# zrlhahaha/Direct12PBRRenderer

Hardware: AMD Instinct MI355X
Metric: shaded Mpixel/s at 4K G-buffer (full deferred frame: clustered shade + bloom + auto-exposure + ACES) (higher is better)
Workload: dtype f32

## Files before the change

direct12pbrrenderer_amd/csrc/bloom.hip:

```cpp
#include <type_traits>
#include "pbr_internal.hpp"
#include "pbr_device.hpp"

using namespace pbr;

__constant__ float c_gauss[9] = {0.0148f, 0.0459f, 0.1050f, 0.1941f, 0.2803f, 0.1941f, 0.1050f, 0.0459f, 0.0148f};

__device__ __forceinline__ float4 to4(F4 v) { return make_float4(v.x, v.y, v.z, v.w); }
__device__ __forceinline__ F4 from4(float4 v) { return f4(v.x, v.y, v.z, v.w); }

struct OutRect { int x0, y0, x1, y1, ox, oy, pitch; };
constexpr int PF_MAX_RECTS = 5;
struct OutRects {
    int n, ox, oy, pitch;
    int x0[PF_MAX_RECTS], y0[PF_MAX_RECTS], x1[PF_MAX_RECTS], y1[PF_MAX_RECTS], tiles_x[PF_MAX_RECTS], first[PF_MAX_RECTS + 1];
};
__global__ __launch_bounds__(256) void k_bloom_prefilter(const pbr_half* __restrict__ hdr, int w, int h, int pitch,
                                                           pbr_half* __restrict__ out, OutRect rc,
                                                           float tx, float ty, float threshold, float knee) {
    const int x = rc.x0 + blockIdx.x * 64 + threadIdx.x;
    const int y = rc.y0 + blockIdx.y * 4 + threadIdx.y;
    if (x >= rc.x1 || y >= rc.y1) return;
    const float u = (float)x * tx, v = (float)y * ty;
    const float ox[5] = {0.0f, -1.0f, -1.0f, 1.0f, 1.0f};
// ... 272 lines not shown
    t.c00 = r0[x0];
    if (MODE != M_SAME) {
        const H4* r1 = reinterpret_cast<const H4*>(in) + (size_t)y1 * iw;
        t.c10 = r0[x1]; t.c01 = r1[x0]; t.c11 = r1[x1];
    }
    return t;
}
template <int MODE>
__device__ __forceinline__ float4 finish_tap2(const Tap2& t, float fx, float fy) {
    if (MODE == M_SAME) return to4(h4f(t.c00));
    const float wx0 = 1.0f - fx, wy0 = 1.0f - fy;
    const F4 top = fma4(h4f(t.c10), fx, h4f(t.c00) * wx0);
    const F4 bot = fma4(h4f(t.c11), fx, h4f(t.c01) * wx0);
    return to4(fma4(bot, fy, top * wy0));
}

typedef _Float16 half4v __attribute__((ext_vector_type(4)));
typedef _Float16 half2v __attribute__((ext_vector_type(2)));
typedef float float2v __attribute__((ext_vector_type(2)));
__device__ __forceinline__ half2v round_h2(float a, float b) {
    asm volatile("" : "+v"(a), "+v"(b));
    float2v f; f.x = a; f.y = b;
    return __builtin_convertvector(f, half2v);
}
__device__ __forceinline__ half4v round_h4(F4 v) {
    half4v r;
    r.x = to_half_rn(v.x); r.y = to_half_rn(v.y); r.z = to_half_rn(v.z); r.w = to_half_rn(v.w);
    return r;
}

__device__ __forceinline__ V3 h3f(H4 h) { return v3((float)h.x, (float)h.y, (float)h.z); }
__device__ __forceinline__ V3 fma3(V3 a, float s, V3 b) { return v3(__builtin_fmaf(a.x, s, b.x), __builtin_fmaf(a.y, s, b.y), __builtin_fmaf(a.z, s, b.z)); }
template <int MODE>
__device__ __forceinline__ float4 finish_tap2_rgb(const Tap2& t, float fx, float fy) {
    if (MODE == M_SAME) return make_float4((float)t.c00.x, (float)t.c00.y, (float)t.c00.z, 0.0f);
    const float wx0 = 1.0f - fx, wy0 = 1.0f - fy;
    const V3 top = fma3(h3f(t.c10), fx, h3f(t.c00) * wx0);
    const V3 bot = fma3(h3f(t.c11), fx, h3f(t.c01) * wx0);
    const V3 r = fma3(bot, fy, top * wy0);
    return make_float4(r.x, r.y, r.z, 0.0f);
}
__device__ __forceinline__ V3 gauss9_rgb(const float4* c) {
    V3 v = v3(0.0f, 0.0f, 0.0f);
#pragma unroll
    for (int i = 0; i < 9; i++) { const float4 e = c[i]; v = fma3(v3(e.x, e.y, e.z), c_gauss[i], v); }
    return v;
}
__device__ __forceinline__ float gauss9_const(float c) {
    float v = 0.0f;
#pragma unroll
    for (int i = 0; i < 9; i++) v = __builtin_fmaf(c, c_gauss[i], v);
    return v;
}

struct TailRect { int tx0, ty0, mx0, my0, mx1, my1, bx, by, hx0, hy0, hx1, hy1; };

template <int MODE, bool DUAL, int TAIL, int TH, int NT>
__global__ __launch_bounds__(NT, 4) void k_blur_hv(const pbr_half* __restrict__ in, int iw, int ih,
                                                 const pbr_half* __restrict__ in2,
                                                 pbr_half* __restrict__ out, int ow, int oh, int out_pitch,
                                                 int tiles_x, int n_tiles,
                                                 TailRect tr, float min_log, float inv_range,
                                                 uint32_t* __restrict__ hist) {
    constexpr int TW = 64, SW = TW + 8, SR = TH + 8;
    constexpr int NW = NT / 64;
    constexpr int PER_T = SR / NW;
    constexpr int PER_O = TH / NW;
    static_assert(SR % NW == 0 && TH % NW == 0 && PER_T * 8 <= 64, "rows must split evenly over the waves; one halo tap per lane");
    __shared__ float4 sLine[DUAL ? 2 : 1][NW][SW];
    __shared__ H4 sT[SR][TW];
    __shared__ uint32_t sh_hist[TAIL == 2 ? NW : 1][TAIL == 2 ? PBR_HISTOGRAM_BINS : 1];
    const int t = threadIdx.x, lane = t & 63;
    const int wv = __builtin_amdgcn_readfirstlane(t >> 6);
    if (TAIL == 2) {
        for (int i = t; i < NW * PBR_HISTOGRAM_BINS; i += NT) (&sh_hist[0][0])[i] = 0u;
    }
    const size_t a_at = MODE == M_UP ? (size_t)min(tr.my0 >> 1, ih - 1) * iw + min(tr.mx0 >> 1, iw - 1) : (size_t)0;
    float alpha_h = gauss9_const((float)reinterpret_cast<const H4*>(in)[a_at].w);
    if (DUAL) alpha_h = alpha_h + gauss9_const((float)reinterpret_cast<const H4*>(in2)[(size_t)min(tr.my0, oh - 1) * ow + min(tr.mx0, ow - 1)].w);
    const h16 alpha_t = to_half_rn(alpha_h);
    const float alpha_v = gauss9_const((float)alpha_t);
    for (int tile = blockIdx.x; tile < n_tiles; tile += gridDim.x) {
    const int x0 = (tr.tx0 + tile % tiles_x) * TW, y0 = (tr.ty0 + tile / tiles_x) * TH;
    const int x = x0 + lane;
    H4 hdr_in[PER_O];
    const bool in_mx = TAIL != 0 && x >= tr.mx0 && x < tr.mx1;
    if (TAIL != 0) {
#pragma unroll
        for (int k = 0; k < PER_O; k++) {
            const int y = y0 + wv + NW * k;
            if (in_mx && y >= tr.my0 && y < tr.my1) hdr_in[k] = *reinterpret_cast<const H4*>(out + 4 * ((size_t)(y - tr.by) * out_pitch + (x - tr.bx)));
        }
    }
    const int r0 = wv * PER_T;
    const bool has_halo = lane < PER_T * 8;
    const int hk = lane >> 3, hc = 64 + (lane & 7);
    float4* line = sLine[0][wv];
    float4* line2 = sLine[DUAL ? 1 : 0][wv];
    auto wave_sync = [] {
        __builtin_amdgcn_fence(__ATOMIC_RELEASE, "wavefront");
        __builtin_amdgcn_wave_barrier();
        __builtin_amdgcn_fence(__ATOMIC_ACQUIRE, "wavefront");
    };
    {
        Tap2 htap;
        H4 up[DUAL ? PER_T : 1], hup;
        float fx, hfx, hfy = 0.0f;
        float4 smp[PER_T];
        int ax0, ax1, bx0, bx1;
        tap1d<MODE>(x0 - 4 + lane, iw, ax0, ax1, fx);
        tap1d<MODE>(x0 - 4 + hc, iw, bx0, bx1, hfx);
        const int sx = clampi(x0 - 4 + lane, 0, ow - 1), shx = clampi(x0 - 4 + hc, 0, ow - 1);
        const int first = y0 - 4 + r0;
        const bool shared_rows = MODE == M_UP && first >= 1 && first + PER_T - 1 <= oh - 2;
        if (MODE == M_UP && shared_rows) {
            constexpr int NR = PER_T / 2 + 2;
            const int base = (first >> 1) - 1 + (first & 1);
            V3 hrow[NR];
            const float wx0 = 1.0f - fx;
#pragma unroll
            for (int j = 0; j < NR; j++) {
                const H4* row = reinterpret_cast<const H4*>(in) + (size_t)min(base + j, ih - 1) * iw;
                const H4 c0 = row[ax0], c1 = row[ax1];
                hrow[j] = fma3(h3f(c1), fx, h3f(c0) * wx0);
            }
            auto blend = [&](auto parity) {
                constexpr int P = decltype(parity)::value;
#pragma unroll
                for (int k = 0; k < PER_T; k++) {
                    constexpr int dummy = 0; (void)dummy;
                    const int odd = (P + k) & 1;
                    const int i0 = (P + k + 1) / 2 - P;
                    const float fyk = odd ? 0.25f : 0.75f, wy0 = 1.0f - fyk;
                    const V3 r = fma3(hrow[i0 + 1], fyk, hrow[i0] * wy0);
                    smp[k] = make_float4(r.x, r.y, r.z, 0.0f);
                }
            };
            if (first & 1) blend(std::integral_constant<int, 1>{}); else blend(std::integral_constant<int, 0>{});
#pragma unroll
            for (int k = 0; k < PER_T; k++)
                if (DUAL) up[k] = reinterpret_cast<const H4*>(in2)[(size_t)(first + k) * ow + sx];
        } else {
            Tap2 taps[PER_T];
            float fy[PER_T];
#pragma unroll
            for (int k = 0; k < PER_T; k++) {
                const int jj = clampi(first + k, 0, oh - 1);
                int ay0, ay1;
                tap1d<MODE>(jj, ih, ay0, ay1, fy[k]);
                taps[k] = load_tap2<MODE>(in, iw, ax0, ax1, ay0, ay1);
                if (DUAL) up[k] = reinterpret_cast<const H4*>(in2)[(size_t)jj * ow + sx];
            }
#pragma unroll
            for (int k = 0; k < PER_T; k++) smp[k] = finish_tap2_rgb<MODE>(taps[k], fx, fy[k]);
        }
        if (has_halo) {
            const int jj = clampi(first + hk, 0, oh - 1);
            int ay0, ay1;
            tap1d<MODE>(jj, ih, ay0, ay1, hfy);
            htap = load_tap2<MODE>(in, iw, bx0, bx1, ay0, ay1);
            if (DUAL) hup = reinterpret_cast<const H4*>(in2)[(size_t)jj * ow + shx];
        }
#pragma unroll
        for (int k = 0; k < PER_T; k++) {
            line[lane] = smp[k];
            if (DUAL) line2[lane] = make_float4((float)up[k].x, (float)up[k].y, (float)up[k].z, 0.0f);
            if (has_halo && hk == k) {
                line[hc] = finish_tap2_rgb<MODE>(htap, hfx, hfy);
                if (DUAL) line2[hc] = make_float4((float)hup.x, (float)hup.y, (float)hup.z, 0.0f);
            }
            wave_sync();
            V3 g = gauss9_rgb(line + lane);
            if (DUAL) g = g + gauss9_rgb(line2 + lane);
            wave_sync();
            H4 th;
            th.x = to_half_rn(g.x); th.y = to_half_rn(g.y); th.z = to_half_rn(g.z); th.w = alpha_t;
            sT[r0 + k][lane] = th;
        }
    }
    __syncthreads();
#pragma unroll
    for (int k = 0; k < PER_O; k++) {
        const int r = wv + NW * k, y = y0 + r;
        if (x >= ow || y >= oh) continue;
        V3 a3 = v3(0.0f, 0.0f, 0.0f);
#pragma unroll
        for (int i = 0; i < 9; i++) a3 = fma3(h3f(sT[r + i][lane]), c_gauss[i], a3);
        const F4 a = f4(a3.x, a3.y, a3.z, alpha_v);
        if (TAIL == 0) {
            store_h4(out + 4 * ((size_t)y * out_pitch + x), a);
        } else {
            if (!(in_mx && y >= tr.my0 && y < tr.my1)) continue;
            const half4v a0 = round_h4(a);
            const F4 s = h4f(hdr_in[k]);
            H4 o;
            o.x = to_half_rn(s.x + (float)a0.x); o.y = to_half_rn(s.y + (float)a0.y); o.z = to_half_rn(s.z + (float)a0.z); o.w = to_half_rn(s.w + (float)a0.w);
            *reinterpret_cast<H4*>(out + 4 * ((size_t)(y - tr.by) * out_pitch + (x - tr.bx))) = o;
            if (TAIL == 2) {
                if (x >= tr.hx0 && x < tr.hx1 && y >= tr.hy0 && y < tr.hy1)
                    atomicAdd(&sh_hist[wv][luminance_bin_exact((float)o.x, (float)o.y, (float)o.z, min_log, inv_range)], 1u);
            }
        }
    }
    if (tile + (int)gridDim.x < n_tiles) __syncthreads();
    }
    if (TAIL == 2) {
        __syncthreads();
        for (int i = t; i < PBR_HISTOGRAM_BINS; i += NT) {
            uint32_t sum = 0;
#pragma unroll
            for (int w2 = 0; w2 < NW; w2++) sum += sh_hist[w2][i];
            if (sum) atomicAdd(&hist[i], sum);
        }
    }
}

__device__ __forceinline__ H4 ld_h4(const void* base, uint32_t byte_off) {
    return *reinterpret_cast<const H4*>(reinterpret_cast<const char*>(base) + byte_off);
}
__device__ __forceinline__ void pair_tap_up(const pbr_half* __restrict__ in, int iw, int cm, int c0, int cp, int ay0, int ay1, float fy,
                                            V3& even, V3& odd) {
    const uint32_t ra = (uint32_t)(ay0 * iw) * 8u, rb = (uint32_t)(ay1 * iw) * 8u, om = (uint32_t)cm * 8u, o0 = (uint32_t)c0 * 8u, op = (uint32_t)cp * 8u;
    const V3 am = h3f(ld_h4(in, ra + om)), a0 = h3f(ld_h4(in, ra + o0)), ap = h3f(ld_h4(in, ra + op));
    const V3 bm = h3f(ld_h4(in, rb + om)), b0 = h3f(ld_h4(in, rb + o0)), bp = h3f(ld_h4(in, rb + op));
    const float wy0 = 1.0f - fy;
    even = fma3(fma3(b0, 0.75f, bm * 0.25f), fy, fma3(a0, 0.75f, am * 0.25f) * wy0);
    odd = fma3(fma3(bp, 0.25f, b0 * 0.75f), fy, fma3(ap, 0.25f, a0 * 0.75f) * wy0);
}
__device__ __forceinline__ void gauss9_pair(const float2* e, float& ge, float& go) {
    const float s[10] = {e[0].x, e[0].y, e[1].x, e[1].y, e[2].x, e[2].y, e[3].x, e[3].y, e[4].x, e[4].y};
    float a = 0.0f, b = 0.0f;
#pragma unroll
    for (int i = 0; i < 9; i++) { a = __builtin_fmaf(s[i], c_gauss[i], a); b = __builtin_fmaf(s[i + 1], c_gauss[i], b); }
    ge = a; go = b;
}

#ifdef PBR_DEBUG_KNOBS
#ifdef PBR_BLOOM_TIMING
__device__ unsigned long long g_tail_stamp[8 * 4096];
#define TSTAMP(i) do { if (TAIL == 2 && t == 0 && tile == (int)blockIdx.x + PBR_BLOOM_TIMING * (int)gridDim.x && blockIdx.x < 4096) g_tail_stamp[blockIdx.x * 8 + (i)] = __builtin_readcyclecounter(); } while (0)
#define TWAIT_VM() asm volatile("s_waitcnt vmcnt(0)" ::: "memory")
extern "C" int pbr_debug_tail_stamps(unsigned long long* host, int n) { return (int)hipMemcpyFromSymbol(host, HIP_SYMBOL(g_tail_stamp), sizeof(unsigned long long) * n); }
#else
#define TSTAMP(i) do {} while (0)
#define TWAIT_VM() do {} while (0)
#endif
template <bool DUAL, int TAIL, int TH>
__global__ __launch_bounds__(512, TH == 16 ? 6 : 4) void k_blur_up_wide(const pbr_half* __restrict__ in, int iw, int ih,
                                                          const pbr_half* __restrict__ in2,
                                                          pbr_half* __restrict__ out, int ow, int oh, int out_pitch,
                                                          int tiles_x, int n_tiles,
                                                          TailRect tr, float min_log, float inv_range,
                                                          uint32_t* __restrict__ hist) {
    constexpr int TW = 128, NP = TW / 2 + 4, SR = TH + 8, NT = 512, NW = NT / 64;
    constexpr int PER_T = SR / NW;
    constexpr int PER_O = TH / 4;
    static_assert(SR % NW == 0 && TH % 4 == 0 && PER_T * 4 <= 64, "rows must split evenly over the waves; one halo pair per lane");
    __shared__ float2 sLine[DUAL ? 2 : 1][NW][3][NP];
    __shared__ H4 sT[SR][TW];
    __shared__ uint32_t sh_hist[TAIL == 2 ? NW : 1][TAIL == 2 ? PBR_HISTOGRAM_BINS : 1];
    const int t = threadIdx.x, lane = t & 63;
    const int wv = __builtin_amdgcn_readfirstlane(t >> 6);
    const int vc = t & 127, vg = __builtin_amdgcn_readfirstlane(t >> 7);
    if (TAIL == 2) {
        for (int i = t; i < NW * PBR_HISTOGRAM_BINS; i += NT) (&sh_hist[0][0])[i] = 0u;
    }
    const size_t a_at = (size_t)min(tr.my0 >> 1, ih - 1) * iw + min(tr.mx0 >> 1, iw - 1);
    float alpha_h = gauss9_const((float)reinterpret_cast<const H4*>(in)[a_at].w);
    if (DUAL) alpha_h = alpha_h + gauss9_const((float)reinterpret_cast<const H4*>(in2)[(size_t)min(tr.my0, oh - 1) * ow + min(tr.mx0, ow - 1)].w);
    const h16 alpha_t = to_half_rn(alpha_h);
    const float alpha_v = gauss9_const((float)alpha_t);
    const float a0w = (float)to_half_rn(alpha_v);
    auto wave_sync = [] {
        __builtin_amdgcn_fence(__ATOMIC_RELEASE, "wavefront");
        __builtin_amdgcn_wave_barrier();
        __builtin_amdgcn_fence(__ATOMIC_ACQUIRE, "wavefront");
    };
    for (int tile = blockIdx.x; tile < n_tiles; tile += gridDim.x) {
    const int x0 = (tr.tx0 + tile % tiles_x) * TW, y0 = (tr.ty0 + tile / tiles_x) * TH;
    const int xv = x0 + vc, rbase = vg * PER_O;
    TSTAMP(0);
    H4 hdr_in[PER_O];
    const bool in_mx = TAIL != 0 && xv >= tr.mx0 && xv < tr.mx1;
    char* const hdr_row0 = reinterpret_cast<char*>(out) + (ptrdiff_t)(y0 + rbase - tr.by) * out_pitch * 8;
    const uint32_t hdr_x = (uint32_t)(xv - tr.bx) * 8u;
    const size_t hdr_pitch = (size_t)out_pitch * 8u;
    const int r0 = wv * PER_T, first = y0 - 4 + r0;
// ... 287 lines not shown
    }
    __syncthreads();
    {
        H4 win[PER_O + 8];
#pragma unroll
        for (int i = 0; i < PER_O + 8; i++) win[i] = sT[rbase + i][vc];
#pragma unroll
        for (int k = 0; k < PER_O; k++) {
            const int y = y0 + rbase + k;
            if (xv >= ow || y >= oh) continue;
            V3 a3 = v3(0.0f, 0.0f, 0.0f);
#pragma unroll
            for (int i = 0; i < 9; i++) a3 = fma3(h3f(win[k + i]), c_gauss[i], a3);
            const F4 a = f4(a3.x, a3.y, a3.z, alpha_v);
            if (TAIL == 0) {
                store_h4(out + 4 * ((size_t)y * out_pitch + xv), a);
            } else {
                if (!(in_mx && y >= tr.my0 && y < tr.my1)) continue;
                const half2v a01 = round_h2(a3.x, a3.y);
                const h16 a2 = to_half_rn(a3.z);
                const F4 s = h4f(hdr_in[k]);
                struct alignas(8) O4 { half2v lo, hi; } o;
                o.lo = round_h2(s.x + (float)a01.x, s.y + (float)a01.y);
                o.hi = round_h2(s.z + (float)a2, s.w + a0w);
                *reinterpret_cast<O4*>(hdr_row0 + k * hdr_pitch + hdr_x) = o;
                if (TAIL == 2) {
                    if (xv >= tr.hx0 && xv < tr.hx1 && y >= tr.hy0 && y < tr.hy1)
                        atomicAdd(&sh_hist[wv][luminance_bin_exact((float)o.lo.x, (float)o.lo.y, (float)o.hi.x, min_log, inv_range)], 1u);
                }
            }
        }
    }
    if (tile + (int)gridDim.x < n_tiles) __syncthreads();
    }
    if (TAIL == 2) {
        __syncthreads();
        for (int i = t; i < PBR_HISTOGRAM_BINS; i += NT) {
            uint32_t sum = 0;
#pragma unroll
            for (int w2 = 0; w2 < NW; w2++) sum += sh_hist[w2][i];
            if (sum) atomicAdd(&hist[i], sum);
        }
    }
}

static int blur_h_rows(uint32_t ow, uint32_t oh) {
    const uint64_t row_blocks = (uint64_t)((ow + 255) / 256) * oh;
    int rows = (int)(row_blocks / 2048);
    return rows < 1 ? 1 : (rows > HB_MAX_ROWS ? HB_MAX_ROWS : rows);
}

static bool exact_half(uint32_t n) { return (n & 1u) == 0u && n <= 8192u; }
static bool force_staged() { static const bool v = pbr::knob_set("PBR_BLOOM_STAGED"); return v; }

template <int MODE, bool DUAL, int TAIL>
static pbr_status launch_hv(pbr_ctx* ctx, const pbr_half* in, uint32_t iw, uint32_t ih, const pbr_half* in2,
                            pbr_half* out, uint32_t ow, uint32_t oh, uint32_t out_pitch,
                            const uint32_t* rect, float min_log, float inv_range, uint32_t* hist,
                            const uint32_t* merge_rect = nullptr, const uint32_t* buf_origin = nullptr) {
    TailRect tr;
    tr.hx0 = rect ? (int)rect[0] : 0; tr.hy0 = rect ? (int)rect[1] : 0;
    tr.hx1 = rect ? (int)(rect[0] + rect[2]) : 0; tr.hy1 = rect ? (int)(rect[1] + rect[3]) : 0;
    tr.mx0 = merge_rect ? (int)merge_rect[0] : 0; tr.my0 = merge_rect ? (int)merge_rect[1] : 0;
    tr.mx1 = merge_rect ? (int)(merge_rect[0] + merge_rect[2]) : (int)ow; tr.my1 = merge_rect ? (int)(merge_rect[1] + merge_rect[3]) : (int)oh;
    tr.bx = buf_origin ? (int)buf_origin[0] : 0; tr.by = buf_origin ? (int)buf_origin[1] : 0;
    static const int hist_blocks = pbr::knob_int("PBR_BLOOM_HIST_BLOCKS", 1024);
    auto even_blocks = [](int n_tiles) { const int per = (n_tiles + hist_blocks - 1) / hist_blocks; return (n_tiles + per - 1) / per; };
    if constexpr (MODE == M_UP) {
        static const int wide_forced = pbr::knob_int("PBR_BLOOM_WIDE", -1);
#ifdef PBR_DEBUG_KNOBS
        static const int wide_th = pbr::knob_int("PBR_BLOOM_WIDE_TH", 32);
#endif
        const int wtx0 = tr.mx0 / 128, wty0 = tr.my0 / 32;
        const int wtiles_x = (tr.mx1 + 127) / 128 - wtx0, wn = wtiles_x * ((tr.my1 + 31) / 32 - wty0);
        if (wide_forced >= 0 ? wide_forced == 1 : (wn >= 400 && !ctx->bloom_shader_order)) {
            tr.tx0 = wtx0; tr.ty0 = wty0;
#ifdef PBR_DEBUG_KNOBS
            static const bool poly_off = pbr::knob_int("PBR_BLOOM_POLY", 1) == 0;
            if (poly_off && wide_th == 16) {
                tr.ty0 = tr.my0 / 16;
                const int wn16 = wtiles_x * ((tr.my1 + 15) / 16 - tr.ty0);
                hipLaunchKernelGGL((k_blur_up_wide<DUAL, TAIL, 16>), dim3(TAIL == 2 ? even_blocks(wn16) : wn16), dim3(512), 0, ctx->stream,
                                   in, (int)iw, (int)ih, in2, out, (int)ow, (int)oh, (int)out_pitch, wtiles_x, wn16, tr, min_log, inv_range, hist);
                return launched(ctx, "k_blur_up_wide<16>");
            }
            if (poly_off) {
                hipLaunchKernelGGL((k_blur_up_wide<DUAL, TAIL, 32>), dim3(TAIL == 2 ? even_blocks(wn) : wn), dim3(512), 0, ctx->stream,
                                   in, (int)iw, (int)ih, in2, out, (int)ow, (int)oh, (int)out_pitch, wtiles_x, wn, tr, min_log, inv_range, hist);
                return launched(ctx, "k_blur_up_wide");
            }
#endif
            hipLaunchKernelGGL((k_blur_up_poly<DUAL, TAIL, 32>), dim3(TAIL == 2 ? even_blocks(wn) : wn), dim3(512), 0, ctx->stream,
                               in, (int)iw, (int)ih, in2, out, (int)ow, (int)oh, (int)out_pitch, wtiles_x, wn, tr, min_log, inv_range, hist);
            return launched(ctx, "k_blur_up_poly");
        }
    }
    static const int forced = pbr::knob_int("PBR_BLOOM_TILE", 0);
    const bool big = forced ? forced == 32 : (uint64_t)((tr.mx1 + 63) / 64 - tr.mx0 / 64) * ((tr.my1 + 31) / 32 - tr.my0 / 32) >= 900;
    const int th = big ? 32 : 16;
    tr.tx0 = tr.mx0 / 64; tr.ty0 = tr.my0 / th;
    const int tiles_x = (tr.mx1 + 63) / 64 - tr.tx0;
    const int n_tiles = tiles_x * ((tr.my1 + th - 1) / th - tr.ty0);
    const int blocks = TAIL == 2 ? even_blocks(n_tiles) : n_tiles;
    if (big) {
        hipLaunchKernelGGL((k_blur_hv<MODE, DUAL, TAIL, 32, 512>), dim3(blocks), dim3(512), 0, ctx->stream,
                           in, (int)iw, (int)ih, in2, out, (int)ow, (int)oh, (int)out_pitch, tiles_x, n_tiles, tr, min_log, inv_range, hist);
    } else if (forced != 16) {
        hipLaunchKernelGGL((k_blur_hv<MODE, DUAL, TAIL, 16, 512>), dim3(blocks), dim3(512), 0, ctx->stream,
                           in, (int)iw, (int)ih, in2, out, (int)ow, (int)oh, (int)out_pitch, tiles_x, n_tiles, tr, min_log, inv_range, hist);
    } else {
        hipLaunchKernelGGL((k_blur_hv<MODE, DUAL, TAIL, 16, 256>), dim3(blocks), dim3(256), 0, ctx->stream,
                           in, (int)iw, (int)ih, in2, out, (int)ow, (int)oh, (int)out_pitch, tiles_x, n_tiles, tr, min_log, inv_range, hist);
    }
    return launched(ctx, "k_blur_hv");
}

extern "C" {

static pbr_status prefilter_launch(pbr_ctx* ctx, const pbr_half* hdr, uint32_t w, uint32_t h, uint32_t pitch,
                                   pbr_half* out, const OutRect* rcs, int n, float threshold, float knee) {
    const uint32_t ow = w >> 1, oh = h >> 1;
    const float tx = 1.0f / (float)ow, ty = 1.0f / (float)oh;
    if (exact_half(w) && exact_half(h) && !force_staged()) {
        OutRects rs{};
        rs.n = n; rs.ox = rcs[0].ox; rs.oy = rcs[0].oy; rs.pitch = rcs[0].pitch;
        int blocks = 0;
        for (int r = 0; r < n; r++) {
            rs.x0[r] = rcs[r].x0; rs.y0[r] = rcs[r].y0; rs.x1[r] = rcs[r].x1; rs.y1[r] = rcs[r].y1;
            rs.tiles_x[r] = (rcs[r].x1 - rcs[r].x0 + PF_TW - 1) / PF_TW;
            rs.first[r] = blocks;
            blocks += rs.tiles_x[r] * ((rcs[r].y1 - rcs[r].y0 + PF_TH - 1) / PF_TH);
        }
        rs.first[n] = blocks;
        hipLaunchKernelGGL(k_bloom_prefilter_2x, dim3(blocks), dim3(256), 0, ctx->stream, hdr, (int)w, (int)h, (int)pitch, out, rs, threshold, knee);
        return launched(ctx, "k_bloom_prefilter_2x");
    }
    for (int r = 0; r < n; r++) {
        const uint32_t rw = (uint32_t)(rcs[r].x1 - rcs[r].x0), rh = (uint32_t)(rcs[r].y1 - rcs[r].y0);
        dim3 grid((rw + 63) / 64, (rh + 3) / 4);
        hipLaunchKernelGGL(k_bloom_prefilter, grid, dim3(64, 4), 0, ctx->stream, hdr, (int)w, (int)h, (int)pitch, out, rcs[r], tx, ty, threshold, knee);
        pbr_status st = launched(ctx, "k_bloom_prefilter");
        if (st) return st;
    }
    return PBR_OK;
}

pbr_status pbr_bloom_prefilter(pbr_ctx* ctx, const pbr_half* hdr, uint32_t w, uint32_t h, uint32_t pitch,
                               pbr_half* out, float threshold, float knee) {
    if (!ctx) return PBR_ERR_INVALID;
    PBR_REQUIRE(ctx, hdr && out, "pbr_bloom_prefilter: null pointer");
    PBR_REQUIRE(ctx, (w >> 1) >= 1 && (h >> 1) >= 1 && w <= 65535 && h <= 65535 && pitch >= w, "pbr_bloom_prefilter: bad size");
// ... 31 lines not shown

pbr_status pbr_blur_h(pbr_ctx* ctx, const pbr_half* in, uint32_t iw, uint32_t ih, pbr_half* out, uint32_t ow, uint32_t oh) {
    if (!ctx) return PBR_ERR_INVALID;
    PBR_REQUIRE(ctx, in && out, "pbr_blur_h: null pointer");
    PBR_REQUIRE(ctx, iw && ih && ow && oh && iw <= 65535 && ih <= 65535 && ow <= 65535 && oh <= 65535, "pbr_blur_h: bad size");
    const float tx = 1.0f / (float)ow, ty = 1.0f / (float)oh;
    const int rows = blur_h_rows(ow, oh);
    dim3 grid((ow + 255) / 256, (oh + rows - 1) / rows);
    hipLaunchKernelGGL(k_blur_h<false>, grid, dim3(256), 0, ctx->stream, in, (int)iw, (int)ih, (const pbr_half*)nullptr, 0, 0, out, (int)ow, (int)oh, tx, ty, rows);
    return launched(ctx, "k_blur_h");
}

pbr_status pbr_blur_v(pbr_ctx* ctx, const pbr_half* in, uint32_t iw, uint32_t ih, pbr_half* out, uint32_t ow, uint32_t oh) {
    if (!ctx) return PBR_ERR_INVALID;
    PBR_REQUIRE(ctx, in && out, "pbr_blur_v: null pointer");
    PBR_REQUIRE(ctx, iw && ih && ow && oh && iw <= 65535 && ih <= 65535 && ow <= 65535 && oh <= 65535, "pbr_blur_v: bad size");
    const float tx = 1.0f / (float)ow, ty = 1.0f / (float)oh;
    dim3 grid((ow + VT_W - 1) / VT_W, (oh + VT_R - 1) / VT_R);
    hipLaunchKernelGGL(k_blur_v, grid, dim3(VT_W, 4), 0, ctx->stream, in, (int)iw, (int)ih, out, (int)ow, (int)oh, tx, ty);
    return launched(ctx, "k_blur_v");
}

pbr_status pbr_bloom_upsample_add(pbr_ctx* ctx, const pbr_half* upper, uint32_t uw, uint32_t uh,
                                  const pbr_half* lower, uint32_t lw, uint32_t lh, pbr_half* out) {
    if (!ctx) return PBR_ERR_INVALID;
    PBR_REQUIRE(ctx, upper && lower && out, "pbr_bloom_upsample_add: null pointer");
    PBR_REQUIRE(ctx, uw && uh && lw && lh && uw <= 65535 && uh <= 65535, "pbr_bloom_upsample_add: bad size");
    const float tx = 1.0f / (float)uw, ty = 1.0f / (float)uh;
    const int rows = blur_h_rows(uw, uh);
    dim3 grid((uw + 255) / 256, (uh + rows - 1) / rows);
    hipLaunchKernelGGL(k_blur_h<true>, grid, dim3(256), 0, ctx->stream, lower, (int)lw, (int)lh, upper, (int)uw, (int)uh, out, (int)uw, (int)uh, tx, ty, rows);
    return launched(ctx, "k_blur_h<dual>");
}

pbr_status pbr_bloom_merge(pbr_ctx* ctx, pbr_half* hdr, uint32_t pitch, const pbr_half* in, uint32_t w, uint32_t h) {
    if (!ctx) return PBR_ERR_INVALID;
    PBR_REQUIRE(ctx, hdr && in, "pbr_bloom_merge: null pointer");
    PBR_REQUIRE(ctx, w && h && w <= 65535 && h <= 65535 && pitch >= w, "pbr_bloom_merge: bad size");
    dim3 grid((w + 255) / 256, h);
    hipLaunchKernelGGL(k_bloom_merge, grid, dim3(256), 0, ctx->stream, hdr, (int)pitch, in, (int)w, (int)h);
    return launched(ctx, "k_bloom_merge");
}

pbr_status pbr_bloom_up_level(pbr_ctx* ctx, const pbr_half* upper, const pbr_half* lower, uint32_t lw, uint32_t lh,
                              pbr_half* out, uint32_t ow, uint32_t oh) {
    if (!ctx) return PBR_ERR_INVALID;
    PBR_REQUIRE(ctx, lower && out && out != lower && out != upper, "pbr_bloom_up_level: null pointer / out aliases an input");
    PBR_REQUIRE(ctx, lw >= 1 && lh >= 1 && ow == 2 * lw && oh == 2 * lh && exact_half(ow) && exact_half(oh), "pbr_bloom_up_level: out must be exactly twice lower, even, <= 8192");
    if (force_staged()) return pbr::fail(ctx, PBR_ERR_UNSUPPORTED, "pbr_bloom_up_level: PBR_BLOOM_STAGED is set");
    if (upper) return launch_hv<M_UP, true, 0>(ctx, lower, lw, lh, upper, out, ow, oh, ow, nullptr, 0.0f, 0.0f, nullptr);
    return launch_hv<M_UP, false, 0>(ctx, lower, lw, lh, nullptr, out, ow, oh, ow, nullptr, 0.0f, 0.0f, nullptr);
}

static pbr_status bloom_final(pbr_ctx* ctx, const pbr_half* b0, pbr_half* hdr, uint32_t w, uint32_t h, uint32_t pitch,
                              const uint32_t* hist_rect, float min_log, float inv_range, uint32_t* hist256) {
    const float tx = 1.0f / (float)w, ty = 1.0f / (float)h;
    const int tiles_x = (int)((w + VT_W - 1) / VT_W), tiles_y = (int)((h + VT_R - 1) / VT_R);
    int blocks = tiles_x * tiles_y;
    if (blocks > 1280) blocks = 1280;
    if (hist256) {
        hipLaunchKernelGGL(k_blur_v_merge<true>, dim3(blocks), dim3(VT_W, 4), 0, ctx->stream, b0, (int)w, (int)h, tx, ty, hdr, (int)pitch, tiles_x, tiles_y,
                           (int)hist_rect[0], (int)hist_rect[1], (int)(hist_rect[0] + hist_rect[2]), (int)(hist_rect[1] + hist_rect[3]), min_log, inv_range, hist256);
    } else {
        hipLaunchKernelGGL(k_blur_v_merge<false>, dim3(blocks), dim3(VT_W, 4), 0, ctx->stream, b0, (int)w, (int)h, tx, ty, hdr, (int)pitch, tiles_x, tiles_y,
                           0, 0, 0, 0, 0.0f, 0.0f, (uint32_t*)nullptr);
    }
    return launched(ctx, "k_blur_v_merge");
}

static pbr_status bloom_pyramid(pbr_ctx* ctx, uint32_t w, uint32_t h, pbr_half* A, pbr_half* B, const pbr_half** res_out, const uint32_t* need0 = nullptr) {
    auto a = [&](uint32_t l) { return A + 4 * pbr_bloom_level_offset(w, h, l); };
    auto b = [&](uint32_t l) { return B + 4 * pbr_bloom_level_offset(w, h, l); };
    auto W = [&](uint32_t l) { return w >> l; };
    auto H = [&](uint32_t l) { return h >> l; };
    pbr_status r;
    auto exact = [&](uint32_t l) { return !force_staged() && exact_half(W(l)) && exact_half(H(l)); };
    for (uint32_t i = 0; i < PBR_BLOOM_STEP; i++) {
        const uint32_t up = i + 1, lo = i + 2;
        if (exact(up)) {
            if ((r = launch_hv<M_DOWN, false, 0>(ctx, a(up), W(up), H(up), nullptr, a(lo), W(lo), H(lo), W(lo), nullptr, 0.0f, 0.0f, nullptr))) return r;
        } else {
            if ((r = pbr_blur_h(ctx, a(up), W(up), H(up), b(lo), W(lo), H(lo)))) return r;
            if ((r = pbr_blur_v(ctx, b(lo), W(lo), H(lo), a(lo), W(lo), H(lo)))) return r;
        }
    }
    uint32_t need[PBR_BLOOM_MIPS][4];
    static const bool shrink = pbr::knob_int("PBR_BLOOM_SHRINK", 1) != 0;
    const bool use_need = need0 != nullptr && shrink;
    if (use_need) {
        int x0 = (int)need0[0], y0 = (int)need0[1], x1 = (int)(need0[0] + need0[2]), y1 = (int)(need0[1] + need0[3]);
        for (uint32_t l = 1; l < PBR_BLOOM_MIPS; l++) {
            x0 = (x0 - 4) / 2 - 2; y0 = (y0 - 4) / 2 - 2; x1 = (x1 + 4 + 1) / 2 + 2; y1 = (y1 + 4 + 1) / 2 + 2;
            const int cx0 = x0 < 0 ? 0 : x0, cy0 = y0 < 0 ? 0 : y0, cx1 = x1 > (int)W(l) ? (int)W(l) : x1, cy1 = y1 > (int)H(l) ? (int)H(l) : y1;
            need[l][0] = (uint32_t)cx0; need[l][1] = (uint32_t)cy0; need[l][2] = (uint32_t)(cx1 - cx0); need[l][3] = (uint32_t)(cy1 - cy0);
            x0 = cx0; y0 = cy0; x1 = cx1; y1 = cy1;
        }
    }
    const pbr_half* res = a(PBR_BLOOM_MIPS - 1);
    for (int i = PBR_BLOOM_STEP - 1; i >= 0; i--) {
        const uint32_t up = (uint32_t)i + 1;
        if (exact(up)) {
            if ((r = launch_hv<M_UP, true, 0>(ctx, res, W(up + 1), H(up + 1), a(up), b(up), W(up), H(up), W(up), nullptr, 0.0f, 0.0f, nullptr,
                                              use_need ? need[up] : nullptr))) return r;
            res = b(up);
        } else {
            if ((r = pbr_bloom_upsample_add(ctx, a(up), W(up), H(up), res, W(up + 1), H(up + 1), b(up)))) return r;
            if ((r = pbr_blur_v(ctx, b(up), W(up), H(up), a(up), W(up), H(up)))) return r;
            res = a(up);
        }
    }
    *res_out = res;
    return PBR_OK;
}

static pbr_status bloom_impl(pbr_ctx* ctx, pbr_half* hdr, uint32_t w, uint32_t h, uint32_t pitch, pbr_half* A, pbr_half* B,
                             float threshold, float knee, const uint32_t* hist_rect, float min_log, float inv_range, uint32_t* hist256) {
    PBR_REQUIRE(ctx, hdr && A && B, "pbr_bloom: null pointer");
    PBR_REQUIRE(ctx, (w >> (PBR_BLOOM_MIPS - 1)) >= 1 && (h >> (PBR_BLOOM_MIPS - 1)) >= 1, "pbr_bloom: image too small for 5 mips");
    PBR_REQUIRE(ctx, w <= 65535 && h <= 65535 && pitch >= w, "pbr_bloom: bad size");
    pbr_status r;
    if ((r = pbr_bloom_prefilter(ctx, hdr, w, h, pitch, A + 4 * pbr_bloom_level_offset(w, h, 1), threshold, knee))) return r;
    const pbr_half* res = nullptr;
    if ((r = bloom_pyramid(ctx, w, h, A, B, &res))) return r;
    if (!force_staged() && exact_half(w) && exact_half(h)) {
        if (hist256) return launch_hv<M_UP, false, 2>(ctx, res, w >> 1, h >> 1, nullptr, hdr, w, h, pitch, hist_rect, min_log, inv_range, hist256);
        return launch_hv<M_UP, false, 1>(ctx, res, w >> 1, h >> 1, nullptr, hdr, w, h, pitch, nullptr, 0.0f, 0.0f, nullptr);
    }
    pbr_half* b0 = B;
    if ((r = pbr_blur_h(ctx, res, w >> 1, h >> 1, b0, w, h))) return r;
    return bloom_final(ctx, b0, hdr, w, h, pitch, hist_rect, min_log, inv_range, hist256);
}

pbr_status pbr_bloom(pbr_ctx* ctx, pbr_half* hdr, uint32_t w, uint32_t h, uint32_t pitch,
                     pbr_half* A, pbr_half* B, float threshold, float knee) {
    if (!ctx) return PBR_ERR_INVALID;
    return bloom_impl(ctx, hdr, w, h, pitch, A, B, threshold, knee, nullptr, 0.0f, 0.0f, nullptr);
}

pbr_status pbr_bloom_histogram(pbr_ctx* ctx, pbr_half* hdr, uint32_t w, uint32_t h, uint32_t pitch,
                               pbr_half* A, pbr_half* B, float threshold, float knee,
                               const uint32_t rect[4], float min_log, float inv_range, uint32_t* hist256) {
    if (!ctx) return PBR_ERR_INVALID;
    PBR_REQUIRE(ctx, rect && hist256, "pbr_bloom_histogram: null pointer");
    PBR_REQUIRE(ctx, rect[2] >= 1 && rect[3] >= 1 && rect[0] + rect[2] <= w && rect[1] + rect[3] <= h, "pbr_bloom_histogram: rect outside the image");
    return bloom_impl(ctx, hdr, w, h, pitch, A, B, threshold, knee, rect, min_log, inv_range, hist256);
}

pbr_status pbr_bloom_tiled(pbr_ctx* ctx, pbr_half* hdr, uint32_t hdr_pitch, const uint32_t hdr_rect[4],
                           uint32_t ew, uint32_t eh, pbr_half* A, pbr_half* B, const uint32_t merge_rect[4],
                           float min_log, float inv_range, uint32_t* hist256) {
    if (!ctx) return PBR_ERR_INVALID;
    PBR_REQUIRE(ctx, hdr && hdr_rect && A && B && merge_rect, "pbr_bloom_tiled: null pointer");
    PBR_REQUIRE(ctx, ew <= 65535 && eh <= 65535 && (ew >> (PBR_BLOOM_MIPS - 1)) >= 1 && (eh >> (PBR_BLOOM_MIPS - 1)) >= 1, "pbr_bloom_tiled: bad size");
    PBR_REQUIRE(ctx, hdr_rect[2] >= 1 && hdr_rect[3] >= 1 && hdr_rect[0] + hdr_rect[2] <= ew && hdr_rect[1] + hdr_rect[3] <= eh && hdr_pitch >= hdr_rect[2],
// ... 16 lines not shown
```

Measured before the change: 17870.

## Fuse pairs of bloom pyramid levels into single down and up kernels

Adds k_blur_down2 and k_blur_up2, which each process two consecutive bloom mip levels in one launch. The intermediate level is kept in LDS, with halo recompute, instead of round-tripping through global memory between launches. This targets launch overhead and the small, low-occupancy launches at the coarse mip levels. In exchange it recomputes overlapping halo regions and uses a large LDS footprint. It is disabled when region shrinking (need) or shader order is active, and the tile-size and poly heuristics now use the full level size rather than the needed rect.

```diff
diff --git a/direct12pbrrenderer_amd/csrc/bloom.hip b/direct12pbrrenderer_amd/csrc/bloom.hip
--- a/direct12pbrrenderer_amd/csrc/bloom.hip
+++ b/direct12pbrrenderer_amd/csrc/bloom.hip
@@ -348,6 +348,31 @@
     for (int i = 0; i < 9; i++) v = __builtin_fmaf(c, c_gauss[i], v);
     return v;
 }
+template <bool DUAL>
+__device__ __forceinline__ V3 hpass_rgb(const float4* line, const float4* line2) {
+    V3 g = gauss9_rgb(line);
+    if (DUAL) g = g + gauss9_rgb(line2);
+    return g;
+}
+__device__ __forceinline__ H4 hround(V3 g, h16 alpha_t) {
+    H4 th;
+    th.x = to_half_rn(g.x); th.y = to_half_rn(g.y); th.z = to_half_rn(g.z); th.w = alpha_t;
+    return th;
+}
+__device__ __forceinline__ V3 vpass_rgb(const H4* col, int stride) {
+    V3 a3 = v3(0.0f, 0.0f, 0.0f);
+#pragma unroll
+    for (int i = 0; i < 9; i++) a3 = fma3(h3f(col[i * stride]), c_gauss[i], a3);
+    return a3;
+}
+struct HvAlpha { h16 t; float v; };
+template <bool DUAL>
+__device__ __forceinline__ HvAlpha hv_alpha(float in_w, float in2_w) {
+    float h = gauss9_const(in_w);
+    if (DUAL) h = h + gauss9_const(in2_w);
+    const h16 t = to_half_rn(h);
+    return HvAlpha{t, gauss9_const((float)t)};
+}
 
 struct TailRect { int tx0, ty0, mx0, my0, mx1, my1, bx, by, hx0, hy0, hx1, hy1; };
 
@@ -372,10 +397,10 @@
         for (int i = t; i < NW * PBR_HISTOGRAM_BINS; i += NT) (&sh_hist[0][0])[i] = 0u;
     }
     const size_t a_at = MODE == M_UP ? (size_t)min(tr.my0 >> 1, ih - 1) * iw + min(tr.mx0 >> 1, iw - 1) : (size_t)0;
-    float alpha_h = gauss9_const((float)reinterpret_cast<const H4*>(in)[a_at].w);
-    if (DUAL) alpha_h = alpha_h + gauss9_const((float)reinterpret_cast<const H4*>(in2)[(size_t)min(tr.my0, oh - 1) * ow + min(tr.mx0, ow - 1)].w);
-    const h16 alpha_t = to_half_rn(alpha_h);
-    const float alpha_v = gauss9_const((float)alpha_t);
+    const HvAlpha al = hv_alpha<DUAL>((float)reinterpret_cast<const H4*>(in)[a_at].w,
+                                      DUAL ? (float)reinterpret_cast<const H4*>(in2)[(size_t)min(tr.my0, oh - 1) * ow + min(tr.mx0, ow - 1)].w : 0.0f);
+    const h16 alpha_t = al.t;
+    const float alpha_v = al.v;
     for (int tile = blockIdx.x; tile < n_tiles; tile += gridDim.x) {
     const int x0 = (tr.tx0 + tile % tiles_x) * TW, y0 = (tr.ty0 + tile / tiles_x) * TH;
     const int x = x0 + lane;
@@ -466,12 +491,9 @@
                 if (DUAL) line2[hc] = make_float4((float)hup.x, (float)hup.y, (float)hup.z, 0.0f);
             }
             wave_sync();
-            V3 g = gauss9_rgb(line + lane);
-            if (DUAL) g = g + gauss9_rgb(line2 + lane);
+            const V3 g = hpass_rgb<DUAL>(line + lane, line2 + lane);
             wave_sync();
-            H4 th;
-            th.x = to_half_rn(g.x); th.y = to_half_rn(g.y); th.z = to_half_rn(g.z); th.w = alpha_t;
-            sT[r0 + k][lane] = th;
+            sT[r0 + k][lane] = hround(g, alpha_t);
         }
     }
     __syncthreads();
@@ -479,9 +501,7 @@
     for (int k = 0; k < PER_O; k++) {
         const int r = wv + NW * k, y = y0 + r;
         if (x >= ow || y >= oh) continue;
-        V3 a3 = v3(0.0f, 0.0f, 0.0f);
-#pragma unroll
-        for (int i = 0; i < 9; i++) a3 = fma3(h3f(sT[r + i][lane]), c_gauss[i], a3);
+        const V3 a3 = vpass_rgb(&sT[r][lane], TW);
         const F4 a = f4(a3.x, a3.y, a3.z, alpha_v);
         if (TAIL == 0) {
             store_h4(out + 4 * ((size_t)y * out_pitch + x), a);
@@ -529,6 +549,244 @@
 #pragma unroll
     for (int i = 0; i < 9; i++) { a = __builtin_fmaf(s[i], c_gauss[i], a); b = __builtin_fmaf(s[i + 1], c_gauss[i], b); }
     ge = a; go = b;
+}
+template <bool DUAL, int NQ>
+__device__ __forceinline__ void hpass_pair_rgb(const float2 (*line)[NQ], const float2 (*line2)[NQ], int q, V3& e, V3& o) {
+    gauss9_pair(line[0] + q, e.x, o.x); gauss9_pair(line[1] + q, e.y, o.y); gauss9_pair(line[2] + q, e.z, o.z);
+    if (DUAL) {
+        V3 ue, uo;
+        gauss9_pair(line2[0] + q, ue.x, uo.x); gauss9_pair(line2[1] + q, ue.y, uo.y); gauss9_pair(line2[2] + q, ue.z, uo.z);
+        e = e + ue; o = o + uo;
+    }
+}
+
+template <int TH>
+__global__ __launch_bounds__(512) void k_blur_up2(const pbr_half* __restrict__ in4, int w4, int h4,
+                                                  const pbr_half* __restrict__ in3, int w3, int h3,
+                                                  const pbr_half* __restrict__ in2, int w2, int h2,
+                                                  pbr_half* __restrict__ out, int tiles_x) {
+    constexpr int NT = 512, TW = 64;
+    constexpr int UC = TW / 2 + 6, UR = TH / 2 + 6;
+    constexpr int AR = UR + 8, AQ = UC / 2 + 4;
+    constexpr int SR = TH + 8, SQ = TW / 2 + 4;
+    static_assert(UC % 2 == 0 && AR * AQ <= NT, "phase A1: one position pair per thread");
+    constexpr size_t A_BYTES = sizeof(float2) * 2 * AR * 3 * AQ + sizeof(H4) * AR * UC, B_BYTES = sizeof(float2) * 2 * SR * 3 * SQ;
+    __shared__ __attribute__((aligned(16))) unsigned char sm[A_BYTES > B_BYTES ? A_BYTES : B_BYTES];
+    __shared__ H4 sU[UR][UC];
+    __shared__ H4 sT[SR][TW];
+    static_assert(sizeof(sm) + sizeof(sU) + sizeof(sT) <= 80 * 1024, "k_blur_up2: two blocks per CU no longer fit the LDS");
+    float2 (*const sA)[3][AQ] = reinterpret_cast<float2 (*)[3][AQ]>(sm);
+    float2 (*const dA)[3][AQ] = sA + AR;
+    H4 (*const tA)[UC] = reinterpret_cast<H4 (*)[UC]>(sm + sizeof(float2) * 2 * AR * 3 * AQ);
+    float2 (*const sB)[3][SQ] = reinterpret_cast<float2 (*)[3][SQ]>(sm);
+    float2 (*const dB)[3][SQ] = sB + SR;
+    const H4* const i3 = reinterpret_cast<const H4*>(in3);
+    const H4* const i2 = reinterpret_cast<const H4*>(in2);
+    const int t = threadIdx.x;
+    const int x0 = (blockIdx.x % tiles_x) * TW, y0 = (blockIdx.x / tiles_x) * TH;
+    const int cx0 = (x0 >> 1) - 3, ry0 = (y0 >> 1) - 3;
+    const HvAlpha al3 = hv_alpha<true>((float)reinterpret_cast<const H4*>(in4)[0].w, (float)i3[0].w);
+    const h16 u_w = to_half_rn(al3.v);
+    const HvAlpha al2 = hv_alpha<true>((float)u_w, (float)i2[0].w);
+
+    constexpr int NB = (SR * SQ + NT - 1) / NT;
+    Tap2 ta[2];
+    H4 da[2], db[NB][2];
+    float fxa[2], fya = 0.0f;
+    const bool a_item = t < AR * AQ;
+    const int ar = t / AQ, aq = t - ar * AQ;
+    if (a_item) {
+        const int j = clampi(ry0 - 4 + ar, 0, h3 - 1);
+        int ay0, ay1;
+        tap1d<M_UP>(j, h4, ay0, ay1, fya);
+#pragma unroll
+        for (int h = 0; h < 2; h++) {
+            const int p = cx0 - 4 + 2 * aq + h;
+            int ax0, ax1;
+            tap1d<M_UP>(p, w4, ax0, ax1, fxa[h]);
+            ta[h] = load_tap2<M_UP>(in4, w4, ax0, ax1, ay0, ay1);
+            da[h] = i3[(size_t)j * w3 + clampi(p, 0, w3 - 1)];
+        }
+    }
+#pragma unroll
+    for (int n = 0; n < NB; n++) {
+        const int e = t + n * NT;
+        if (e >= SR * SQ) break;
+        const int k = e / SQ, q = e - k * SQ;
+        const H4* row = i2 + (size_t)clampi(y0 - 4 + k, 0, h2 - 1) * w2;
+        db[n][0] = row[clampi(x0 - 4 + 2 * q, 0, w2 - 1)];
+        db[n][1] = row[clampi(x0 - 3 + 2 * q, 0, w2 - 1)];
+    }
+    if (a_item) {
+        const float4 e0 = finish_tap2_rgb<M_UP>(ta[0], fxa[0], fya), e1 = finish_tap2_rgb<M_UP>(ta[1], fxa[1], fya);
+        sA[ar][0][aq] = make_float2(e0.x, e1.x); sA[ar][1][aq] = make_float2(e0.y, e1.y); sA[ar][2][aq] = make_float2(e0.z, e1.z);
+        dA[ar][0][aq] = make_float2((float)da[0].x, (float)da[1].x); dA[ar][1][aq] = make_float2((float)da[0].y, (float)da[1].y);
+        dA[ar][2][aq] = make_float2((float)da[0].z, (float)da[1].z);
+    }
+    __syncthreads();
+    for (int e = t; e < AR * (UC / 2); e += NT) {
+        const int r = e / (UC / 2), q = e - r * (UC / 2);
+        V3 ge, go;
+        hpass_pair_rgb<true>(sA[r], dA[r], q, ge, go);
+        tA[r][2 * q] = hround(ge, al3.t);
+        tA[r][2 * q + 1] = hround(go, al3.t);
+    }
+    __syncthreads();
+    for (int e = t; e < UR * UC; e += NT) {
+        const int r = e / UC, c = e - r * UC;
+        const V3 a3 = vpass_rgb(&tA[r][c], UC);
+        H4 u;
+        u.x = to_half_rn(a3.x); u.y = to_half_rn(a3.y); u.z = to_half_rn(a3.z); u.w = u_w;
+        sU[r][c] = u;
+    }
+    __syncthreads();
+#pragma unroll
+    for (int n = 0; n < NB; n++) {
+        const int e = t + n * NT;
+        if (e >= SR * SQ) break;
+        const int k = e / SQ, q = e - k * SQ;
+        int iy0, iy1;
+        float fy;
+        tap1d<M_UP>(clampi(y0 - 4 + k, 0, h2 - 1), h3, iy0, iy1, fy);
+        iy0 -= ry0; iy1 -= ry0;
+        float4 smp[2];
+#pragma unroll
+        for (int h = 0; h < 2; h++) {
+            int ix0, ix1;
+            float fx;
+            tap1d<M_UP>(x0 - 4 + 2 * q + h, w3, ix0, ix1, fx);
+            ix0 -= cx0; ix1 -= cx0;
+            const Tap2 tp{sU[iy0][ix0], sU[iy0][ix1], sU[iy1][ix0], sU[iy1][ix1]};
+            smp[h] = finish_tap2_rgb<M_UP>(tp, fx, fy);
+        }
+        sB[k][0][q] = make_float2(smp[0].x, smp[1].x); sB[k][1][q] = make_float2(smp[0].y, smp[1].y); sB[k][2][q] = make_float2(smp[0].z, smp[1].z);
+        dB[k][0][q] = make_float2((float)db[n][0].x, (float)db[n][1].x); dB[k][1][q] = make_float2((float)db[n][0].y, (float)db[n][1].y);
+        dB[k][2][q] = make_float2((float)db[n][0].z, (float)db[n][1].z);
+    }
+    __syncthreads();
+    for (int e = t; e < SR * (TW / 2); e += NT) {
+        const int k = e / (TW / 2), q = e - k * (TW / 2);
+        V3 ge, go;
+        hpass_pair_rgb<true>(sB[k], dB[k], q, ge, go);
+        sT[k][2 * q] = hround(ge, al2.t);
+        sT[k][2 * q + 1] = hround(go, al2.t);
+    }
+    __syncthreads();
+    for (int e = t; e < TH * TW; e += NT) {
+        const int r = e / TW, x = x0 + (e - r * TW), y = y0 + r;
+        if (x >= w2 || y >= h2) continue;
+        const V3 a3 = vpass_rgb(&sT[r][x - x0], TW);
+        store_h4(out + 4 * ((size_t)y * w2 + x), f4(a3.x, a3.y, a3.z, al2.v));
+    }
+}
+
+template <int TW, int TH>
+__global__ __launch_bounds__(512) void k_blur_down2(const pbr_half* __restrict__ in2, int w2, int h2,
+                                                    pbr_half* __restrict__ out3, int w3, int h3,
+                                                    pbr_half* __restrict__ out4, int w4, int h4,
+                                                    int tiles_x) {
+    constexpr int NT = 512;
+    static_assert(TW % 4 == 0 && TH % 2 == 0, "level-(L+2) texels in column pairs");
+    constexpr int RC = TW + 16, RR = TH + 16;
+    constexpr int AR = RR + 8, AQ = RC / 2 + 4;
+    constexpr int OW = TW / 2, OH = TH / 2;
+    constexpr int BR = OH + 8, BQ = OW / 2 + 4;
+    constexpr size_t SA_BYTES = sizeof(float2) * AR * 3 * AQ, R_BYTES = sizeof(H4) * RR * RC;
+    constexpr size_t TA_BYTES = sizeof(H4) * AR * RC, B_BYTES = sizeof(float2) * BR * 3 * BQ + sizeof(H4) * BR * OW;
+    __shared__ __attribute__((aligned(16))) unsigned char sm0[SA_BYTES > R_BYTES ? SA_BYTES : R_BYTES];
+    __shared__ __attribute__((aligned(16))) unsigned char sm1[TA_BYTES > B_BYTES ? TA_BYTES : B_BYTES];
+    static_assert(sizeof(sm0) + sizeof(sm1) <= 80 * 1024, "k_blur_down2: two blocks per CU no longer fit the LDS");
+    float2 (*const sA)[3][AQ] = reinterpret_cast<float2 (*)[3][AQ]>(sm0);
+    H4 (*const sR)[RC] = reinterpret_cast<H4 (*)[RC]>(sm0);
+    H4 (*const tA)[RC] = reinterpret_cast<H4 (*)[RC]>(sm1);
+    float2 (*const sB)[3][BQ] = reinterpret_cast<float2 (*)[3][BQ]>(sm1);
+    H4 (*const tB)[OW] = reinterpret_cast<H4 (*)[OW]>(sm1 + sizeof(float2) * BR * 3 * BQ);
+    const int t = threadIdx.x;
+    const int x0 = (blockIdx.x % tiles_x) * TW, y0 = (blockIdx.x / tiles_x) * TH;
+    const int rx0 = x0 - 8, ry0 = y0 - 8, x40 = x0 >> 1, y40 = y0 >> 1;
+    const HvAlpha al3 = hv_alpha<false>((float)reinterpret_cast<const H4*>(in2)[0].w, 0.0f);
+    const h16 r_w = to_half_rn(al3.v);
+    const HvAlpha al4 = hv_alpha<false>((float)r_w, 0.0f);
+
+    constexpr int NA = (AR * AQ + NT - 1) / NT;
+    Tap2 ta[NA][2];
+#pragma unroll
+    for (int n = 0; n < NA; n++) {
+        const int e = t + n * NT;
+        if (e >= AR * AQ) break;
+        const int r = e / AQ, q = e - r * AQ;
+        int ay0, ay1;
+        float fy;
+        tap1d<M_DOWN>(clampi(ry0 - 4 + r, 0, h3 - 1), h2, ay0, ay1, fy);
+#pragma unroll
+        for (int h = 0; h < 2; h++) {
+            int ax0, ax1;
+            float fx;
+            tap1d<M_DOWN>(rx0 - 4 + 2 * q + h, w2, ax0, ax1, fx);
+            ta[n][h] = load_tap2<M_DOWN>(in2, w2, ax0, ax1, ay0, ay1);
+        }
+    }
+#pragma unroll
+    for (int n = 0; n < NA; n++) {
+        const int e = t + n * NT;
+        if (e >= AR * AQ) break;
+        const int r = e / AQ, q = e - r * AQ;
+        const float4 e0 = finish_tap2_rgb<M_DOWN>(ta[n][0], 0.5f, 0.5f), e1 = finish_tap2_rgb<M_DOWN>(ta[n][1], 0.5f, 0.5f);
+        sA[r][0][q] = make_float2(e0.x, e1.x); sA[r][1][q] = make_float2(e0.y, e1.y); sA[r][2][q] = make_float2(e0.z, e1.z);
+    }
+    __syncthreads();
+    for (int e = t; e < AR * (RC / 2); e += NT) {
+        const int r = e / (RC / 2), q = e - r * (RC / 2);
+        V3 ge, go;
+        hpass_pair_rgb<false>(sA[r], sA[r], q, ge, go);
+        tA[r][2 * q] = hround(ge, al3.t);
+        tA[r][2 * q + 1] = hround(go, al3.t);
+    }
+    __syncthreads();
+    for (int e = t; e < RR * RC; e += NT) {
+        const int r = e / RC, c = e - r * RC;
+        const V3 a3 = vpass_rgb(&tA[r][c], RC);
+        H4 v;
+        v.x = to_half_rn(a3.x); v.y = to_half_rn(a3.y); v.z = to_half_rn(a3.z); v.w = r_w;
+        sR[r][c] = v;
+        const int x = rx0 + c, y = ry0 + r;
+        if (x >= x0 && x < x0 + TW && y >= y0 && y < y0 + TH && x < w3 && y < h3)
+            *reinterpret_cast<H4*>(out3 + 4 * ((size_t)y * w3 + x)) = v;
+    }
+    __syncthreads();
+    for (int e = t; e < BR * BQ; e += NT) {
+        const int k = e / BQ, q = e - k * BQ;
+        int iy0, iy1;
+        float fy;
+        tap1d<M_DOWN>(clampi(y40 - 4 + k, 0, h4 - 1), h3, iy0, iy1, fy);
+        iy0 -= ry0; iy1 -= ry0;
+        float4 smp[2];
+#pragma unroll
+        for (int h = 0; h < 2; h++) {
+            int ix0, ix1;
+            float fx;
+            tap1d<M_DOWN>(x40 - 4 + 2 * q + h, w3, ix0, ix1, fx);
+            ix0 -= rx0; ix1 -= rx0;
+            const Tap2 tp{sR[iy0][ix0], sR[iy0][ix1], sR[iy1][ix0], sR[iy1][ix1]};
+            smp[h] = finish_tap2_rgb<M_DOWN>(tp, fx, fy);
+        }
+        sB[k][0][q] = make_float2(smp[0].x, smp[1].x); sB[k][1][q] = make_float2(smp[0].y, smp[1].y); sB[k][2][q] = make_float2(smp[0].z, smp[1].z);
+    }
+    __syncthreads();
+    for (int e = t; e < BR * (OW / 2); e += NT) {
+        const int k = e / (OW / 2), q = e - k * (OW / 2);
+        V3 ge, go;
+        hpass_pair_rgb<false>(sB[k], sB[k], q, ge, go);
+        tB[k][2 * q] = hround(ge, al4.t);
+        tB[k][2 * q + 1] = hround(go, al4.t);
+    }
+    __syncthreads();
+    for (int e = t; e < OH * OW; e += NT) {
+        const int r = e / OW, x = x40 + (e - r * OW), y = y40 + r;
+        if (x >= w4 || y >= h4) continue;
+        const V3 a3 = vpass_rgb(&tB[r][x - x40], OW);
+        store_h4(out4 + 4 * ((size_t)y * w4 + x), f4(a3.x, a3.y, a3.z, al4.v));
+    }
 }
 
 #ifdef PBR_DEBUG_KNOBS
@@ -922,6 +1180,12 @@
 
 static bool exact_half(uint32_t n) { return (n & 1u) == 0u && n <= 8192u; }
 static bool force_staged() { static const bool v = pbr::knob_set("PBR_BLOOM_STAGED"); return v; }
+static bool fuse_level_pairs() { static const bool v = pbr::knob_int("PBR_BLOOM_FUSE", 1) != 0; return v; }
+static bool up_level_poly(const pbr_ctx* ctx, uint32_t ow, uint32_t oh) {
+    static const int wide_forced = pbr::knob_int("PBR_BLOOM_WIDE", -1);
+    const uint64_t wn = (uint64_t)((ow + 127) / 128) * ((oh + 31) / 32);
+    return wide_forced >= 0 ? wide_forced == 1 : (wn >= 400 && !ctx->bloom_shader_order);
+}
 
 template <int MODE, bool DUAL, int TAIL>
 static pbr_status launch_hv(pbr_ctx* ctx, const pbr_half* in, uint32_t iw, uint32_t ih, const pbr_half* in2,
@@ -937,13 +1201,12 @@
     static const int hist_blocks = pbr::knob_int("PBR_BLOOM_HIST_BLOCKS", 1024);
     auto even_blocks = [](int n_tiles) { const int per = (n_tiles + hist_blocks - 1) / hist_blocks; return (n_tiles + per - 1) / per; };
     if constexpr (MODE == M_UP) {
-        static const int wide_forced = pbr::knob_int("PBR_BLOOM_WIDE", -1);
 #ifdef PBR_DEBUG_KNOBS
         static const int wide_th = pbr::knob_int("PBR_BLOOM_WIDE_TH", 32);
 #endif
         const int wtx0 = tr.mx0 / 128, wty0 = tr.my0 / 32;
         const int wtiles_x = (tr.mx1 + 127) / 128 - wtx0, wn = wtiles_x * ((tr.my1 + 31) / 32 - wty0);
-        if (wide_forced >= 0 ? wide_forced == 1 : (wn >= 400 && !ctx->bloom_shader_order)) {
+        if (up_level_poly(ctx, ow, oh)) {
             tr.tx0 = wtx0; tr.ty0 = wty0;
 #ifdef PBR_DEBUG_KNOBS
             static const bool poly_off = pbr::knob_int("PBR_BLOOM_POLY", 1) == 0;
@@ -966,7 +1229,7 @@
         }
     }
     static const int forced = pbr::knob_int("PBR_BLOOM_TILE", 0);
-    const bool big = forced ? forced == 32 : (uint64_t)((tr.mx1 + 63) / 64 - tr.mx0 / 64) * ((tr.my1 + 31) / 32 - tr.my0 / 32) >= 900;
+    const bool big = forced ? forced == 32 : (uint64_t)((ow + 63) / 64) * ((oh + 31) / 32) >= 900;
     const int th = big ? 32 : 16;
     tr.tx0 = tr.mx0 / 64; tr.ty0 = tr.my0 / th;
     const int tiles_x = (tr.mx1 + 63) / 64 - tr.tx0;
@@ -1104,6 +1367,24 @@
     return launch_hv<M_UP, false, 0>(ctx, lower, lw, lh, nullptr, out, ow, oh, ow, nullptr, 0.0f, 0.0f, nullptr);
 }
 
+static pbr_status launch_down2(pbr_ctx* ctx, const pbr_half* in2, uint32_t w2, uint32_t h2, pbr_half* out3, uint32_t w3, uint32_t h3,
+                               pbr_half* out4, uint32_t w4, uint32_t h4) {
+    constexpr int TW = 32, TH = 16;
+    const int tiles_x = (int)((w3 + TW - 1) / TW), n_tiles = tiles_x * (int)((h3 + TH - 1) / TH);
+    hipLaunchKernelGGL((k_blur_down2<TW, TH>), dim3(n_tiles), dim3(512), 0, ctx->stream, in2, (int)w2, (int)h2, out3, (int)w3, (int)h3,
+                       out4, (int)w4, (int)h4, tiles_x);
+    return launched(ctx, "k_blur_down2");
+}
+
+static pbr_status launch_up2(pbr_ctx* ctx, const pbr_half* in4, uint32_t w4, uint32_t h4, const pbr_half* in3, uint32_t w3, uint32_t h3,
+                             const pbr_half* in2, pbr_half* out, uint32_t w2, uint32_t h2) {
+    constexpr int TH = 16;
+    const int tiles_x = (int)((w2 + 63) / 64), n_tiles = tiles_x * (int)((h2 + TH - 1) / TH);
+    hipLaunchKernelGGL(k_blur_up2<TH>, dim3(n_tiles), dim3(512), 0, ctx->stream, in4, (int)w4, (int)h4, in3, (int)w3, (int)h3,
+                       in2, (int)w2, (int)h2, out, tiles_x);
+    return launched(ctx, "k_blur_up2");
+}
+
 static pbr_status bloom_final(pbr_ctx* ctx, const pbr_half* b0, pbr_half* hdr, uint32_t w, uint32_t h, uint32_t pitch,
                               const uint32_t* hist_rect, float min_log, float inv_range, uint32_t* hist256) {
     const float tx = 1.0f / (float)w, ty = 1.0f / (float)h;
@@ -1127,8 +1408,15 @@
     auto H = [&](uint32_t l) { return h >> l; };
     pbr_status r;
     auto exact = [&](uint32_t l) { return !force_staged() && exact_half(W(l)) && exact_half(H(l)); };
+    static const bool shrink = pbr::knob_int("PBR_BLOOM_SHRINK", 1) != 0;
+    const bool use_need = need0 != nullptr && shrink;
+    const bool fuse = fuse_level_pairs() && !ctx->bloom_shader_order && !use_need;
     for (uint32_t i = 0; i < PBR_BLOOM_STEP; i++) {
         const uint32_t up = i + 1, lo = i + 2;
+        if (fuse && i + 2 == PBR_BLOOM_STEP && exact(up) && exact(lo)) {
+            if ((r = launch_down2(ctx, a(up), W(up), H(up), a(lo), W(lo), H(lo), a(lo + 1), W(lo + 1), H(lo + 1)))) return r;
+            break;
+        }
         if (exact(up)) {
             if ((r = launch_hv<M_DOWN, false, 0>(ctx, a(up), W(up), H(up), nullptr, a(lo), W(lo), H(lo), W(lo), nullptr, 0.0f, 0.0f, nullptr))) return r;
         } else {
@@ -1137,8 +1425,6 @@
         }
     }
     uint32_t need[PBR_BLOOM_MIPS][4];
-    static const bool shrink = pbr::knob_int("PBR_BLOOM_SHRINK", 1) != 0;
-    const bool use_need = need0 != nullptr && shrink;
     if (use_need) {
         int x0 = (int)need0[0], y0 = (int)need0[1], x1 = (int)(need0[0] + need0[2]), y1 = (int)(need0[1] + need0[3]);
         for (uint32_t l = 1; l < PBR_BLOOM_MIPS; l++) {
@@ -1149,9 +1435,16 @@
         }
     }
     const pbr_half* res = a(PBR_BLOOM_MIPS - 1);
+    auto fused_pair = [&](uint32_t up) {
+        return fuse && up >= 2 && exact(up) && exact(up - 1) && !up_level_poly(ctx, W(up), H(up)) && !up_level_poly(ctx, W(up - 1), H(up - 1));
+    };
     for (int i = PBR_BLOOM_STEP - 1; i >= 0; i--) {
         const uint32_t up = (uint32_t)i + 1;
-        if (exact(up)) {
+        if (fused_pair(up)) {
+            if ((r = launch_up2(ctx, res, W(up + 1), H(up + 1), a(up), W(up), H(up), a(up - 1), b(up - 1), W(up - 1), H(up - 1)))) return r;
+            res = b(up - 1);
+            i--;
+        } else if (exact(up)) {
             if ((r = launch_hv<M_UP, true, 0>(ctx, res, W(up + 1), H(up + 1), a(up), b(up), W(up), H(up), W(up), nullptr, 0.0f, 0.0f, nullptr,
                                               use_need ? need[up] : nullptr))) return r;
             res = b(up);
```

Result: faster. 18060 (median of 6 runs) (+1.0%).
